# Illumina/canvas

Hardware: AMD Instinct MI355X
Metric: genome-bins/sec (bin+clean+partition) (higher is better)
Workload: dtype u8/int32 (bin), f32/f64 (clean, viterbi); 1 GPU; BASELINE configs[2]: whole-genome GRCh38 60x single sample, full bin+clean+partition HIP path on 1 MI355X per sample; bins_after_clean=4686240, bin_size=534, partition=PerSampleHMM, clean_flags=-g -s -r --local-sd-metric-file, segments=250, samples=1

## Files before the change

### canvas_amd/csrc/hmm.hip

```cpp
#include "common.hpp"
#include <type_traits>
#include "select.hpp"
#include "quantize.hpp"
#include <mutex>
#include <cmath>
#include <thread>
#include <cstring>
#include <limits>
#include <algorithm>

#define NSTATE 5

struct HmmParams {
    double logA[NSTATE][NSTATE];
    double logPi[NSTATE];
    int32_t tableLen;
    double maxThreshold;
};

__global__ void __launch_bounds__(256) k_keys_cov_f32(const double* __restrict__ cov, int64_t n, uint32_t* __restrict__ keys) {
    int64_t i = (int64_t)blockIdx.x * 256 + threadIdx.x;
    if (i < n) keys[i] = key_of_float((float)cov[i]);
}

// ... 409 lines not shown
#pragma unroll
            for (int j = 0; j < NSTATE; j++) { d[j] = on ? dn[j] : d[j]; eCur[j] = eNext[j]; }
            if (WM) { fm = (on && s >= lead) ? map_compose(fm, pk) : fm; pks[u] = pk; }
        }
        if (WM) {
#pragma unroll
            for (int u = 0; u < PQ; u++) { const int s = s0 + u; if (s < nsteps && s >= lead) pp[ts + s] = (uint16_t)pks[u]; }
        }
        qa = na; qb = nb;
    };
    const int leadMin = -wave_max_i32(nsteps > 0 ? -lead : -0x7FFFFFFF);
    int s0 = 1;
    for (; s0 + PQ <= leadMin && s0 < maxSteps; s0 += PQ) group(s0, std::false_type{});
    for (; s0 < maxSteps; s0 += PQ) group(s0, std::true_type{});
    if (act) {
        maps[b] = (uint16_t)fm;
        if (tEnd == C.T) lastGuess[B.chrom] = vit_best5(d);
    }
}

#define CHR_LDS_CAP 1024
__device__ __forceinline__ const int64_t* stage_chr_offsets(const int64_t* __restrict__ chrOff, int nchr, int64_t* sOff) {
    if (nchr + 1 > CHR_LDS_CAP) return chrOff;
    for (int k = threadIdx.x; k <= nchr; k += blockDim.x) sOff[k] = chrOff[k];
    __syncthreads();
    return sOff;
}
__device__ __forceinline__ int chrom_of_bin(const int64_t* off, int nchr, int64_t g) {
    int lo = 0, hi = nchr - 1;
    while (lo < hi) { const int mid = (lo + hi + 1) >> 1; if (off[mid] <= g) lo = mid; else hi = mid - 1; }
    return lo;
}
#define VBS (VB / 2)
__global__ void __launch_bounds__(256) k_pair_maps(const VitBlock* __restrict__ blocks, int nblocks, const HmmChrom* __restrict__ chroms, const int32_t* __restrict__ firstS,
                                                   const uint16_t* __restrict__ mapsS, uint16_t* __restrict__ maps, const int32_t* __restrict__ todo) {
    const int b = blockIdx.x * 256 + threadIdx.x;
    if (b >= nblocks) return;
    const VitBlock B = blocks[b];
    if (todo && !todo[B.chrom]) return;
    const int64_t T = chroms[B.chrom].T;
    const int s0 = firstS[B.chrom] + B.t0 / VBS;
    uint32_t m = mapsS[s0];
#pragma unroll
    for (int k = 1; k < VB / VBS; k++) if (B.t0 + (int64_t)k * VBS < T) m = map_compose(m, mapsS[s0 + k]);
    maps[b] = (uint16_t)m;
}

__global__ void __launch_bounds__(256) k_vit_increments(const HmmChrom* __restrict__ chroms, int nchr, const int64_t* __restrict__ chrOff, const int32_t* __restrict__ idx,
                                                        const double* __restrict__ logPmf, HmmParams P, const int32_t* __restrict__ state, int64_t N, double* __restrict__ D) {
    __shared__ int64_t sOff[CHR_LDS_CAP];
    const int64_t* off = stage_chr_offsets(chrOff, nchr, sOff);
    int64_t g = (int64_t)blockIdx.x * 256 + threadIdx.x;
    if (g >= N) return;
    const int s1 = state[g], sPrev = state[g > 0 ? g - 1 : 0], ix = idx[g];
    const int lo = chrom_of_bin(off, nchr, g);
    const int64_t begin = chroms[lo].begin;
    if (s1 < 0) { D[g] = 0.0; return; }
    double e = logPmf[(size_t)s1 * P.tableLen + ix];
    if (g == begin) { double lik = e + P.logA[0][s1]; D[g] = P.logPi[s1] + lik - P.logA[0][s1]; }
    else { const int s0 = sPrev; D[g] = e + P.logA[s0 < 0 ? 0 : s0][s1]; }
}

__global__ void __launch_bounds__(64) k_vit_backbone(const HmmChrom* __restrict__ chroms, const double* __restrict__ V, double* __restrict__ carryOut, const int32_t* __restrict__ todo = nullptr) {
    __shared__ double sV[2][64];
    const HmmChrom C = chroms[blockIdx.x];
    if (C.T <= 10 || (todo && !todo[blockIdx.x])) return;
    const int l = threadIdx.x;
    const double* __restrict__ Vc = V + C.begin;
    double acc = 0.0;
    double vNext = l < C.T ? Vc[l] : 0.0;
    int buf = 0;
    for (int64_t c0 = 0; c0 < C.T; c0 += 64, buf ^= 1) {
        sV[buf][l] = vNext;
        { int64_t t2 = c0 + 64 + l; vNext = t2 < C.T ? Vc[t2] : 0.0; }
        if (l == 0) carryOut[C.begin + c0] = acc;
        double r[64];
#pragma unroll
        for (int s = 0; s < 64; s++) r[s] = sV[buf][s];
#pragma unroll
        for (int s = 0; s < 64; s++) acc = acc + r[s];
    }
}

#define BS_T 1024
#define BS_I 8
struct ParFn { unsigned long long a0, a1; };
__device__ __forceinline__ ParFn parfn_then(ParFn f, ParFn g) {
    ParFn h;
    h.a0 = f.a0 + ((f.a0 & 1ull) ? g.a1 : g.a0);
    h.a1 = f.a1 + ((f.a1 & 1ull) ? g.a0 : g.a1);
    return h;
}
__device__ __forceinline__ ParFn parfn_shfl_up(ParFn f, int d) {
// ... 93 lines not shown
        }
        __syncthreads();
        if (cross < chunkEnd && myCross == cross) {
            const double Mprev = __longlong_as_double((long long)(expBits | (kBefore & MANT)));
            const double acc = -Mprev + Vc[cross];
            if (((cross + 1) & 63) == 0 && cross + 1 < C.T) carry[cross + 1] = acc;
            sM = -acc; sP = cross + 1; sCross = 0x7fffffffffffffffll;
        }
        __syncthreads();
    }
}

#define BB_CHUNK 1024
#define BB_MAXC 16
struct BbChunk { int32_t chrom; int32_t t0; };
struct BbCross { ParFn before; double v; int32_t pos; int32_t e; };
struct BbChunkOut { ParFn tail; int32_t nCross; int32_t headE; int64_t pad; };
struct BbPost { unsigned long long bits; };
__device__ __forceinline__ bool bb_bad_increment(unsigned long long vb) { return ((vb >> 52) & 0x7ffull) == 0x7ffull || (!(vb >> 63) && (vb << 1) != 0ull); }
__device__ __forceinline__ ParFn parfn_of(unsigned long long vb, int eM) {
    const unsigned long long MANT = (1ull << 52) - 1ull;
    const int ea = (int)((vb >> 52) & 0x7ffull);
    const unsigned long long ma = ea ? ((vb & MANT) | (1ull << 52)) : (vb & MANT);
    const int shift = eM - (ea ? ea : 1);
    unsigned long long A = 0; int r = 0;
    if (shift <= 0) { if (ma) A = 1ull << 53; }
    else if (shift < 64) { A = ma >> shift; const unsigned long long rem = ma & ((1ull << shift) - 1ull), half = 1ull << (shift - 1); r = rem > half ? 1 : (rem == half ? 2 : 0); }
    const unsigned long long up = A + (r == 1 ? 1ull : 0ull);
    ParFn f; f.a0 = up + ((r == 2 && (A & 1ull)) ? 1ull : 0ull); f.a1 = up + ((r == 2 && !(A & 1ull)) ? 1ull : 0ull);
    return f;
}
__device__ __forceinline__ double shfl_up_f64(double v, int d) { return __hiloint2double(__shfl_up(__double2hiint(v), d), __shfl_up(__double2loint(v), d)); }

__global__ void __launch_bounds__(256) k_bb_sums(const BbChunk* __restrict__ chunks, const HmmChrom* __restrict__ chroms, const double* __restrict__ V, double* __restrict__ chunkSum,
                                                 int32_t* __restrict__ fail) {
    __shared__ double sw[4];
    const BbChunk K = chunks[blockIdx.x];
    const HmmChrom C = chroms[K.chrom];
    const double* __restrict__ Vc = V + C.begin;
    double s = 0.0; bool bad = false;
#pragma unroll
    for (int i = 0; i < 4; i++) {
        const int64_t t = (int64_t)K.t0 + threadIdx.x * 4 + i;
        if (t < C.T) { const double v = Vc[t]; bad |= bb_bad_increment((unsigned long long)__double_as_longlong(v)); s += fabs(v); }
    }
#pragma unroll
    for (int d = 32; d >= 1; d >>= 1) s += __hiloint2double(__shfl_xor(__double2hiint(s), d), __shfl_xor(__double2loint(s), d));
    if ((threadIdx.x & 63) == 0) sw[threadIdx.x >> 6] = s;
    if (bad) fail[K.chrom] = 1;
    __syncthreads();
    if (threadIdx.x == 0) chunkSum[blockIdx.x] = (sw[0] + sw[1]) + (sw[2] + sw[3]);
}
__global__ void __launch_bounds__(64) k_bb_bases(const int32_t* __restrict__ firstChunk, const double* __restrict__ chunkSum, double* __restrict__ chunkBase) {
    const int c = blockIdx.x, l = threadIdx.x;
    double carry = 0.0;
    for (int g = firstChunk[c]; g < firstChunk[c + 1]; g += 64) {
        const int i = g + l;
        const double v = i < firstChunk[c + 1] ? chunkSum[i] : 0.0;
        double inc = v;
#pragma unroll
        for (int d = 1; d < 64; d <<= 1) { double o = shfl_up_f64(inc, d); if (l >= d) inc += o; }
        if (i < firstChunk[c + 1]) chunkBase[i] = carry + (inc - v);
        carry += __hiloint2double(__builtin_amdgcn_readlane(__double2hiint(inc), 63), __builtin_amdgcn_readlane(__double2loint(inc), 63));
    }
}
struct SegFn { ParFn f; uint32_t head; uint32_t cnt; };
__device__ __forceinline__ SegFn segfn_then(SegFn a, SegFn b) {
    SegFn r; r.head = a.head | b.head; r.cnt = a.cnt + b.cnt; r.f = b.head ? b.f : parfn_then(a.f, b.f);
    return r;
}
__global__ void __launch_bounds__(256) k_bb_pieces(const BbChunk* __restrict__ chunks, const HmmChrom* __restrict__ chroms, const double* __restrict__ V,
                                                   const double* __restrict__ chunkBase, BbChunkOut* __restrict__ outChunk, BbCross* __restrict__ outCross,
                                                   ParFn* __restrict__ at64Fn, uint8_t* __restrict__ at64Rank, int32_t* __restrict__ fail) {
    __shared__ double swSum[4];
    __shared__ SegFn swSeg[4];
    const BbChunk K = chunks[blockIdx.x];
    const HmmChrom C = chroms[K.chrom];
// ... 282 lines not shown
            double e[NSTATE];
            vit_emissions(e, sTab, logPmf, useLds, P.tableLen, ix[0]);
            const double Dt = S.Dprev + Vc[0];
            const int sCur = st[0];
            vit_init5(S.d, e, P); S.valid = 31u;
            if (sel5(S.d, (uint32_t)sCur) != Dt) { S.bad = true; S.why |= 16u; }
            S.Dprev = Dt; S.sPrev = sCur;
        } else ver_lead_step<useLds>(S, A, sTab, logPmf, P.tableLen, true, ix[0], st[0], Vc[0], (uint32_t)pp[0]);
    }
    const int start2 = lead > 1 ? lead : 1;
    ver_phase<useLds, true>(S, A, P, sTab, logPmf, ix + 1, st + 1, Vc + 1, pp + 1, nsteps > 0 && lead > 1 ? lead - 1 : 0);
    ver_phase<useLds, false>(S, A, P, sTab, logPmf, ix + start2, st + start2, Vc + start2, pp + start2, nsteps > start2 ? nsteps - start2 : 0);
    double (&d)[NSTATE] = S.d; const uint32_t valid = S.valid; bool bad = S.bad;
    uint32_t why = S.why;
    if (act && tEnd == C.T) { if (valid != 31u || vit_best5(d) != lastGuess[B.chrom]) { bad = true; why |= 32u; } }
    if (act && bad) atomicOr(&fail[B.chrom], (int32_t)(1u | why));
}

__global__ void k_vit_corrupt(uint16_t* __restrict__ psi, int64_t at, int j) {
    if (threadIdx.x == 0 && blockIdx.x == 0) { const uint32_t sh = 3u * (uint32_t)j; uint32_t v = psi[at], p = (v >> sh) & 7u; psi[at] = (uint16_t)((v & ~(7u << sh)) | (((p + 1u) % 5u) << sh)); }
}

__global__ void __launch_bounds__(256) k_bt_maps(const VitBlock* __restrict__ blocks, int nblocks, const HmmChrom* __restrict__ chroms, const uint16_t* __restrict__ psi,
                                                 uint16_t* __restrict__ maps) {
    int b = blockIdx.x * 256 + threadIdx.x;
    if (b >= nblocks) return;
    const VitBlock B = blocks[b];
    const HmmChrom C = chroms[B.chrom];
    const int64_t tBeg = B.t0 > 0 ? B.t0 : 1, tEnd = (B.t0 + VB < C.T) ? B.t0 + VB : C.T;
    uint32_t m = MAP_IDENT;
    for (int64_t t = tEnd - 1; t >= tBeg; t--) m = map_compose(psi[C.begin + t], m);
    maps[b] = (uint16_t)m;
}
__global__ void __launch_bounds__(64) k_bt_group(const int32_t* __restrict__ firstBlock, const int32_t* __restrict__ firstGroup, int nchr, const uint16_t* __restrict__ maps,
                                                 uint16_t* __restrict__ pre, uint16_t* __restrict__ gmap) {
    const int g = blockIdx.x, l = threadIdx.x;
    int lo = 0, hi = nchr - 1;
    while (lo < hi) { const int mid = (lo + hi + 1) >> 1; if (firstGroup[mid] <= g) lo = mid; else hi = mid - 1; }
    while (lo < nchr - 1 && firstGroup[lo + 1] <= g) lo++;
    const int first = firstBlock[lo], last = firstBlock[lo + 1] - 1;
    const int bi = last - ((g - firstGroup[lo]) * 64 + l);
    uint32_t f = bi >= first ? (uint32_t)maps[bi] : MAP_IDENT;
#pragma unroll
    for (int dlt = 1; dlt < 64; dlt <<= 1) { const uint32_t o = __shfl_up(f, dlt); if (l >= dlt) f = map_compose(f, o); }
    const uint32_t ex = __shfl_up(f, 1);
    if (bi >= first) pre[bi] = (uint16_t)(l == 0 ? MAP_IDENT : ex);
    if (l == 63) gmap[g] = (uint16_t)f;
}
__global__ void __launch_bounds__(64) k_bt_gchain(const int32_t* __restrict__ firstGroup, const int32_t* __restrict__ lastState, const uint16_t* __restrict__ gmap,
                                                  int8_t* __restrict__ gentry) {
    const int c = blockIdx.x, l = threadIdx.x;
    const int g0 = firstGroup[c], ng = firstGroup[c + 1] - g0;
    int s = lastState[c];
    for (int base = 0; base < ng; base += 64) {
        uint32_t f = base + l < ng ? (uint32_t)gmap[g0 + base + l] : MAP_IDENT;
#pragma unroll
        for (int dlt = 1; dlt < 64; dlt <<= 1) { const uint32_t o = __shfl_up(f, dlt); if (l >= dlt) f = map_compose(f, o); }
        const uint32_t ex = __shfl_up(f, 1);
        if (base + l < ng) gentry[g0 + base + l] = (int8_t)(s < 0 ? s : (l == 0 ? s : (int)map_get(ex, (uint32_t)s)));
        const uint32_t all = (uint32_t)__builtin_amdgcn_readlane((int)f, 63);
        if (s >= 0) s = (int)map_get(all, (uint32_t)s);
    }
}
__global__ void __launch_bounds__(256) k_bt_states(const VitBlock* __restrict__ blocks, int nblocks, const HmmChrom* __restrict__ chroms, const uint16_t* __restrict__ psi,
                                                   const int32_t* __restrict__ firstBlock, const int32_t* __restrict__ firstGroup, const uint16_t* __restrict__ pre,
                                                   const int8_t* __restrict__ gentry, int32_t* __restrict__ state) {
    static_assert(VB <= 128, "two steps per lane");
    const int b = blockIdx.x * 4 + (threadIdx.x >> 6), l = lane_id();
    if (b >= nblocks) return;
    const VitBlock B = blocks[b];
    const HmmChrom C = chroms[B.chrom];
    const int64_t tBeg = B.t0, tEnd = (B.t0 + VB < C.T) ? B.t0 + VB : C.T;
    const int cnt = (int)(tEnd - tBeg);
    const int sg = gentry[firstGroup[B.chrom] + (firstBlock[B.chrom + 1] - 1 - b) / 64];
    const int s = sg < 0 ? sg : (int)map_get((uint32_t)pre[b], (uint32_t)sg);
// ... 285 lines not shown
        L.firstBlock[c] = L.nblocks;
        if (L.chroms[c].T > 10) L.nblocks += (int)((L.chroms[c].T + VB - 1) / VB);
    }
    L.firstBlock[nchr] = L.nblocks;
    L.firstGroup.resize(nchr + 1);
    for (int c = 0; c < nchr; c++) { L.firstGroup[c] = L.ngroups; L.ngroups += (L.firstBlock[c + 1] - L.firstBlock[c] + 63) / 64; }
    L.firstGroup[nchr] = L.ngroups;
    L.firstS.resize(nchr + 1);
    for (int c = 0; c < nchr; c++) { L.firstS[c] = L.nblocksS; if (L.chroms[c].T > 10) L.nblocksS += (int)((L.chroms[c].T + VBS - 1) / VBS); }
    L.firstS[nchr] = L.nblocksS;
    L.firstChunk.resize(nchr + 1);
    for (int c = 0; c < nchr; c++) {
        L.firstChunk[c] = L.nchunks;
        if (L.chroms[c].T > 10) L.nchunks += (int)((L.chroms[c].T + BB_CHUNK - 1) / BB_CHUNK);
    }
    L.firstChunk[nchr] = L.nchunks;
    return L;
}

enum { BB_MODE_CHAIN = 0, BB_MODE_SCAN = 1, BB_MODE_PIECES = 2 };
struct BbWork { double* chunkSum; double* chunkBase; BbChunkOut* chunkOut; BbCross* cross; ParFn* at64Fn; uint8_t* at64Rank; unsigned long long* chunkBits; BbPost* post; };
static void bb_work_size(WsSizer& sz, int nchunks) {
    sz.take<double>(nchunks + 1); sz.take<double>(nchunks + 1); sz.take<BbChunkOut>(nchunks + 1);
    sz.take<BbCross>((size_t)nchunks * BB_MAXC + 1); sz.take<ParFn>((size_t)nchunks * 16 + 1); sz.take<uint8_t>((size_t)nchunks * 16 + 8);
    sz.take<unsigned long long>(nchunks + 1); sz.take<BbPost>((size_t)nchunks * BB_MAXC + 1);
}
static BbWork bb_work_carve(WsCarver& ws, int nchunks) {
    BbWork W;
    W.chunkSum = ws.take<double>(nchunks + 1); W.chunkBase = ws.take<double>(nchunks + 1); W.chunkOut = ws.take<BbChunkOut>(nchunks + 1);
    W.cross = ws.take<BbCross>((size_t)nchunks * BB_MAXC + 1); W.at64Fn = ws.take<ParFn>((size_t)nchunks * 16 + 1); W.at64Rank = ws.take<uint8_t>((size_t)nchunks * 16 + 8);
    W.chunkBits = ws.take<unsigned long long>(nchunks + 1); W.post = ws.take<BbPost>((size_t)nchunks * BB_MAXC + 1);
    return W;
}
static void enqueue_backbone(canvas_ctx* ctx, int mode, int nchr, int nchunks, const HmmChrom* dChroms, const BbChunk* dBChunks, const int32_t* dFirstChunk, const double* dV,
                             double* dCarry, int32_t* dFail, const int32_t* dTodo, const BbWork& W) {
    if (mode == BB_MODE_CHAIN) hipLaunchKernelGGL(k_vit_backbone, dim3(nchr), dim3(64), 0, ctx->stream, dChroms, dV, dCarry, dTodo);
    else if (mode == BB_MODE_SCAN) hipLaunchKernelGGL(k_vit_backbone_scan, dim3(nchr), dim3(BS_T), 0, ctx->stream, dChroms, dV, dCarry, dFail);
    else {
        hipLaunchKernelGGL(k_bb_sums, dim3(nchunks), dim3(256), 0, ctx->stream, dBChunks, dChroms, dV, W.chunkSum, dFail);
        hipLaunchKernelGGL(k_bb_bases, dim3(nchr), dim3(64), 0, ctx->stream, dFirstChunk, W.chunkSum, W.chunkBase);
        hipLaunchKernelGGL(k_bb_pieces, dim3(nchunks), dim3(256), 0, ctx->stream, dBChunks, dChroms, dV, W.chunkBase, W.chunkOut, W.cross, W.at64Fn, W.at64Rank, dFail);
        hipLaunchKernelGGL(k_bb_walk, dim3(nchr), dim3(64), 0, ctx->stream, dFirstChunk, W.chunkOut, W.cross, W.chunkBits, W.post, dFail);
        hipLaunchKernelGGL(k_bb_emit, dim3(nblk2((int64_t)nchunks * 16, 256)), dim3(256), 0, ctx->stream, dBChunks, nchunks, dChroms, W.chunkBits, W.post, W.at64Fn, W.at64Rank, dCarry);
    }
}

struct VitCorrupt { bool on = false, retry = false; int chrom = 0; int64_t t = 0; int state = 2; int attempts = 0; };
static int32_t vit_corrupt_parse(canvas_ctx* ctx, int32_t nchr, const int64_t* h_chr_offset, VitCorrupt& K) {
    const char* s = cvx_hook("CANVAS_HMM_TEST_CORRUPT");
    if (!s) return CANVAS_OK;
    K.on = true;
    if (!strcmp(s, "1")) {
        const int64_t T = h_chr_offset[1] - h_chr_offset[0];
        K.chrom = 0; K.t = T / 2; K.state = 2; K.attempts = T > 10 ? 1 : 0;
        return CANVAS_OK;
    }
    long long v[4] = {0, 0, 0, 0}; int nf = 0; const char* p = s;
    for (;;) {
        char* end = nullptr;
        if (nf == 4 || *p < '0' || *p > '9') { nf = -1; break; }
        v[nf++] = strtoll(p, &end, 10);
        if (end - p > 12) { nf = -1; break; }
        if (*end == 0) break;
        if (*end != ':') { nf = -1; break; }
        p = end + 1;
    }
    if (nf != 3 && nf != 4) CANVAS_FAIL(ctx, CANVAS_ERR_INVALID, "CANVAS_HMM_TEST_CORRUPT: 1, c:t:j or c:t:j:k");
    if (v[0] >= nchr) CANVAS_FAIL(ctx, CANVAS_ERR_INVALID, "CANVAS_HMM_TEST_CORRUPT: no such chromosome");
    const int64_t T = h_chr_offset[v[0] + 1] - h_chr_offset[v[0]];
    if (T <= 10 || v[1] < 1 || v[1] >= T) CANVAS_FAIL(ctx, CANVAS_ERR_INVALID, "CANVAS_HMM_TEST_CORRUPT: the step must be 1 .. T-1 of a chromosome of more than ten bins");
    if (v[2] >= NSTATE) CANVAS_FAIL(ctx, CANVAS_ERR_INVALID, "CANVAS_HMM_TEST_CORRUPT: the state must be 0 .. 4");
    if (nf == 4 && (v[3] < 1 || v[3] > 5)) CANVAS_FAIL(ctx, CANVAS_ERR_INVALID, "CANVAS_HMM_TEST_CORRUPT: 1 .. 5 corrupted attempts");
    K.chrom = (int)v[0]; K.t = v[1]; K.state = (int)v[2]; K.attempts = nf == 4 ? (int)v[3] : 1; K.retry = nf == 4;
    return CANVAS_OK;
}

struct HmmEmis { int32_t* idx = nullptr; double* dTab = nullptr;
                 const double* indexCov = nullptr; };
struct SegPost { const int32_t* d_start; const int32_t* d_stop; int32_t maxDist; int32_t* d_segment_id; int64_t nseg = 0; bool valid = false; };
static void enqueue_segment_ids(canvas_ctx* ctx, const int64_t* dOff, int nchr, const int32_t* d_state, const int32_t* d_start, const int32_t* d_stop, int64_t N, int32_t maxDist,
                                uint8_t* flags, uint32_t* blockCnt, unsigned long long* dTot, int32_t* d_segment_id, unsigned* totSeq = nullptr, unsigned seq = 0);
template <class PrepareA, class PrepareB>
static int32_t hmm_pipeline(canvas_ctx* ctx, int32_t nchr, const int64_t* h_chr_offset, size_t extraBytes, PrepareA prepareA, PrepareB prepareB, int32_t* d_state, SegPost* seg = nullptr,
                            bool descByValue = false ) {
    const int64_t N = h_chr_offset[nchr];
    VitCorrupt corrupt;
    { int32_t rcc = vit_corrupt_parse(ctx, nchr, h_chr_offset, corrupt); if (rcc) return rcc; }
    const HmmLists L = hmm_lists(nchr, h_chr_offset);
    const std::vector<HmmChrom>& chroms = L.chroms;
    const std::vector<int32_t>&firstBlock = L.firstBlock, &firstGroup = L.firstGroup, &firstS = L.firstS, &firstChunk = L.firstChunk;
    const int nblocks = L.nblocks, ngroups = L.ngroups, nblocksS = L.nblocksS, nchunks = L.nchunks;
    const int nbSeg = (int)nblk2(N, 2048);
    WsSizer sz;
    sz.take<BbChunk>(nchunks + 1); sz.take<int32_t>(nchr + 1); bb_work_size(sz, nchunks);
    sz.take<uint16_t>(N + 8); sz.take<HmmChrom>(nchr); sz.take<int32_t>(nchr);
    sz.take<int32_t>(nchr + 1); sz.take<uint16_t>(nblocks + 8); sz.take<int8_t>(nblocks + 8);
    sz.take<int64_t>(nchr + 1); sz.take<VitBlock>(nblocks + 1); sz.take<double>(N); sz.take<double>(N + 64); sz.take<int32_t>(nchr); sz.take<int32_t>(nchr);
    sz.take<VitBlock>(nblocksS + 1); sz.take<uint16_t>(nblocksS + 8); sz.take<int32_t>(nchr + 1);
    sz.take<int32_t>(nchr + 1); sz.take<uint16_t>(nblocks + 8); sz.take<uint16_t>(ngroups + 8); sz.take<int8_t>(ngroups + 8);
    sz.take<char>(8 * 256 + (size_t)nchr * 64 + 64);
    if (seg) { sz.take<uint8_t>(N + 16); sz.take<uint32_t>(nbSeg + 1); sz.take<unsigned long long>(1); }
    int32_t rc = canvas_ws_reserve(ctx, sz.off + extraBytes + 65536); if (rc) return rc;
    rc = canvas_pin_reserve(ctx, (size_t)nchr * 4 + 64); if (rc) return rc;
    WsCarver ws(ctx->ws);
    uint16_t* psi = ws.take<uint16_t>(N + 8);
    HmmChrom* dChroms = ws.take<HmmChrom>(nchr); int32_t* dLast = ws.take<int32_t>(nchr);
    int32_t* dFirst = ws.take<int32_t>(nchr + 1);
    uint16_t* dMaps = ws.take<uint16_t>(nblocks + 8); (void)ws.take<int8_t>(nblocks + 8);
    int64_t* dOffDev = ws.take<int64_t>(nchr + 1);
    VitBlock* dVBlocks = ws.take<VitBlock>(nblocks + 1); double* dD = ws.take<double>(N); double* dCarry = ws.take<double>(N + 64); int32_t* dFail = ws.take<int32_t>(nchr); int32_t* dRedo = ws.take<int32_t>(nchr);
    int32_t* dFirstGroup = ws.take<int32_t>(nchr + 1); uint16_t* dPre = ws.take<uint16_t>(nblocks + 8); uint16_t* dGmap = ws.take<uint16_t>(ngroups + 8);
    int8_t* dGentry = ws.take<int8_t>(ngroups + 8);
    VitBlock* dSBlocks = ws.take<VitBlock>(nblocksS + 1); uint16_t* dMapsS = ws.take<uint16_t>(nblocksS + 8); int32_t* dFirstS = ws.take<int32_t>(nchr + 1);
    BbChunk* dBChunks = ws.take<BbChunk>(nchunks + 1); int32_t* dFirstChunk = ws.take<int32_t>(nchr + 1);
// ... 12 lines not shown
            memset(&pack, 0, sizeof pack);
            memcpy(pack.chroms, chroms.data(), (size_t)nchr * sizeof(HmmChrom)); memcpy(pack.off, h_chr_offset, (size_t)(nchr + 1) * 8); memcpy(pack.first, firstBlock.data(), (size_t)(nchr + 1) * 4);
            memcpy(pack.firstChunk, firstChunk.data(), (size_t)(nchr + 1) * 4); memcpy(pack.firstS, firstS.data(), (size_t)(nchr + 1) * 4); memcpy(pack.firstGroup, firstGroup.data(), (size_t)(nchr + 1) * 4);
        } else {
            std::vector<char> blob(total, 0);
            memcpy(blob.data() + oCh, chroms.data(), (size_t)nchr * sizeof(HmmChrom)); memcpy(blob.data() + oFirst, firstBlock.data(), (size_t)(nchr + 1) * 4);
            memcpy(blob.data() + oOff, h_chr_offset, (size_t)(nchr + 1) * 8); memcpy(blob.data() + oChunk, firstChunk.data(), (size_t)(nchr + 1) * 4);
            memcpy(blob.data() + oS, firstS.data(), (size_t)(nchr + 1) * 4); memcpy(blob.data() + oG, firstGroup.data(), (size_t)(nchr + 1) * 4);
            rc = canvas_h2d_small(ctx, dBlob, blob.data(), total); if (rc) return rc;
        }
        dChroms = (HmmChrom*)(dBlob + oCh); dFirst = (int32_t*)(dBlob + oFirst); dOffDev = (int64_t*)(dBlob + oOff); dFirstChunk = (int32_t*)(dBlob + oChunk);
        dFirstS = (int32_t*)(dBlob + oS); dFirstGroup = (int32_t*)(dBlob + oG);
    }
    HmmParams P; HmmEmis E;
    ctx->hmm_dispersion = 1e9;
    rc = prepareA(ws, P, E, (const HmmChrom*)dChroms, (const int64_t*)dOffDev); if (rc) return rc;
    {
        const int64_t most = std::max<int64_t>(std::max<int64_t>(E.indexCov ? N : 0, nblocks), std::max<int64_t>(std::max(nblocksS, nchunks), nchr));
        HmmDescDev DD{dChroms, dOffDev, dFirst, dFirstChunk, dFirstS, dFirstGroup};
        hipLaunchKernelGGL((k_hmm_setup<VitBlock, BbChunk>), dim3(nblk2(most, 256)), dim3(256), 0, ctx->stream, pack, byVal ? 1 : 0, DD, nchr, nblocks, nblocksS, nchunks, VB, VBS, BB_CHUNK,
                           dVBlocks, dSBlocks, dBChunks, E.indexCov, N, P.maxThreshold, E.idx, dLast, dFail);
    }
    rc = prepareB(ws, P, E); if (rc) return rc;
    int32_t* idx = E.idx; double* dTab = E.dTab;
    size_t tabBytes = (size_t)NSTATE * P.tableLen * 8;
    size_t lds = tabBytes <= 48 * 1024 ? tabBytes : 0;
    for (int c = 0; c < nchr; c++)
        if (chroms[c].T <= 10 && chroms[c].T > 0)
            hipLaunchKernelGGL(k_fill_i32, dim3(nblk2(chroms[c].T, 256)), dim3(256), 0, ctx->stream, d_state, chroms[c].begin, chroms[c].begin + chroms[c].T, -1);
    const unsigned laneGrid = (unsigned)((nblocks + 63) / 64);
    auto backtrack = [&](bool haveMaps) {
        if (nblocks > 0) {
            if (!haveMaps) hipLaunchKernelGGL(k_bt_maps, dim3(nblk2(nblocks, 256)), dim3(256), 0, ctx->stream, dVBlocks, nblocks, dChroms, psi, dMaps);
            hipLaunchKernelGGL(k_bt_group, dim3(ngroups), dim3(64), 0, ctx->stream, dFirst, dFirstGroup, nchr, dMaps, dPre, dGmap);
            hipLaunchKernelGGL(k_bt_gchain, dim3(nchr), dim3(64), 0, ctx->stream, dFirstGroup, dLast, dGmap, dGentry);
            hipLaunchKernelGGL(k_bt_states, dim3(nblk2(nblocks, 4)), dim3(256), 0, ctx->stream, dVBlocks, nblocks, dChroms, psi, dFirst, dFirstGroup, dPre, dGentry, d_state);
        }
    };
    bool twoValuedAll = true;
    for (int i = 0; i < NSTATE; i++) for (int j = 0; j < NSTATE; j++) {
        const double ref = i == j ? P.logA[0][0] : P.logA[0][1];
        if (memcmp(&P.logA[i][j], &ref, sizeof(double)) != 0) twoValuedAll = false;
    }
    const bool speculative = cvx_hook("CANVAS_HMM_SEQUENTIAL") == nullptr;
    std::vector<int32_t> redo;
    int32_t* hFail = (int32_t*)ctx->pin; unsigned long long* hSegTot = (unsigned long long*)((char*)ctx->pin + (((size_t)nchr * 4 + 15) & ~size_t(15)));
    bool segEnqueued = false; unsigned* hSegSeq = (unsigned*)(hSegTot + 1); unsigned segSeq = 0;
    if (speculative && nblocks > 0) {
        ProfScope ps(ctx, "viterbi");
        const int32_t* dTodo = nullptr;
        ctx->hmm_retry = 0;
        const int vwEnv = cvx_hook("CANVAS_HMM_LEAD") ? atoi(cvx_hook("CANVAS_HMM_LEAD")) : 0;
        const int vw0 = vwEnv > 0 ? vwEnv : (ctx->hmm_dispersion < 0.20 ? VW0 : (ctx->hmm_dispersion < 0.30 ? 64 : VW));
        const int nAttempts = 5;
        for (int attempt = 0; attempt < nAttempts; attempt++) {
            const int mult = attempt <= 1 ? 1 : (attempt == 2 ? 8 : (attempt == 3 ? 64 : 512));
            const int leadSpec = attempt == 0 ? vw0 : mult * VW, leadVer = mult * VW2;
            cvx_prof_count(ctx, "viterbi_attempt");
            if (attempt > 0) CANVAS_HIP_TRY(ctx, hipMemsetAsync(dFail, 0, nchr * 4, ctx->stream));
            const dim3 gs((unsigned)((nblocksS + 63) / 64));
            const bool twoValued = twoValuedAll && attempt < 3;
            if (lds && twoValued) hipLaunchKernelGGL((k_vit_spec<true, true>), gs, dim3(64), lds, ctx->stream, dSBlocks, nblocksS, dChroms, idx, dTab, P, psi, dMapsS, dLast, leadSpec, dTodo, VBS);
            else if (lds) hipLaunchKernelGGL((k_vit_spec<true, false>), gs, dim3(64), lds, ctx->stream, dSBlocks, nblocksS, dChroms, idx, dTab, P, psi, dMapsS, dLast, leadSpec, dTodo, VBS);
            else if (twoValued) hipLaunchKernelGGL((k_vit_spec<false, true>), gs, dim3(64), 0, ctx->stream, dSBlocks, nblocksS, dChroms, idx, dTab, P, psi, dMapsS, dLast, leadSpec, dTodo, VBS);
            else hipLaunchKernelGGL((k_vit_spec<false, false>), gs, dim3(64), 0, ctx->stream, dSBlocks, nblocksS, dChroms, idx, dTab, P, psi, dMapsS, dLast, leadSpec, dTodo, VBS);
            hipLaunchKernelGGL(k_pair_maps, dim3(nblk2(nblocks, 256)), dim3(256), 0, ctx->stream, dVBlocks, nblocks, dChroms, dFirstS, dMapsS, dMaps, dTodo);
            if (attempt < corrupt.attempts) hipLaunchKernelGGL(k_vit_corrupt, dim3(1), dim3(64), 0, ctx->stream, psi, chroms[corrupt.chrom].begin + corrupt.t, corrupt.state);
            backtrack(true);
            hipLaunchKernelGGL(k_vit_increments, dim3(nblk2(N, 256)), dim3(256), 0, ctx->stream, dChroms, nchr, dOffDev, idx, dTab, P, d_state, N, dD);
            const char* bbMode = cvx_hook("CANVAS_HMM_BACKBONE");
            const int bb = ((bbMode && !strcmp(bbMode, "chain")) || (attempt > 1 && !bbMode)) ? BB_MODE_CHAIN : ((bbMode && !strcmp(bbMode, "scan")) ? BB_MODE_SCAN : BB_MODE_PIECES);
            enqueue_backbone(ctx, bb, nchr, nchunks, dChroms, dBChunks, dFirstChunk, dD, dCarry, dFail, dTodo, bbWork);
            if (lds) hipLaunchKernelGGL((k_vit_verify<true>), dim3(laneGrid), dim3(64), lds, ctx->stream, dVBlocks, nblocks, dChroms, idx, dTab, P, psi, d_state, dD, dCarry, dLast, dFail, leadVer, dTodo);
            else hipLaunchKernelGGL((k_vit_verify<false>), dim3(laneGrid), dim3(64), 0, ctx->stream, dVBlocks, nblocks, dChroms, idx, dTab, P, psi, d_state, dD, dCarry, dLast, dFail, leadVer, dTodo);
            CANVAS_HIP_TRY(ctx, hipMemcpyAsync(hFail, dFail, nchr * 4, hipMemcpyDeviceToHost, ctx->stream));
            if (seg && attempt == 0 && (!corrupt.on || corrupt.retry)) {
                (void)segTot;
                segSeq = cvx_mail_arm(ctx, hSegSeq);
                enqueue_segment_ids(ctx, dOffDev, nchr, d_state, seg->d_start, seg->d_stop, N, seg->maxDist, segFlags, segBlockCnt, hSegTot , seg->d_segment_id, hSegSeq, segSeq);
                segEnqueued = true;
            }
            CANVAS_HIP_TRY(ctx, hipStreamSynchronize(ctx->stream));
            redo.clear();
            for (int c = 0; c < nchr; c++) if (hFail[c] && chroms[c].T > 10) redo.push_back(c);
            if (!redo.empty() && cvx_hook("CANVAS_HMM_DEBUG_FAIL")) { fprintf(stderr, "viterbi attempt %d (lead-in x%d):", attempt, mult); for (int c : redo) fprintf(stderr, " chr%d(T=%lld, why=0x%x)", c, (long long)chroms[c].T, (unsigned)hFail[c]); fprintf(stderr, "\n"); }
            if (redo.empty() || (corrupt.on && !corrupt.retry) || cvx_hook("CANVAS_HMM_NO_RETRY")) break;
            if (attempt < nAttempts - 1) {
                if (attempt == 0) { ctx->hmm_retry = (int)redo.size(); { ProfScope pr(ctx, "viterbi_retry"); } }
                int32_t rcq = canvas_h2d_small(ctx, dRedo, hFail, nchr * 4); if (rcq) return rcq;
                dTodo = dRedo;
            }
        }
        if (seg && segEnqueued && redo.empty() && ctx->hmm_retry == 0) { int32_t rcm = cvx_mail_await(ctx, hSegSeq, segSeq, "PerSampleHMM: segment count"); if (rcm) return rcm; seg->valid = true; seg->nseg = (int64_t)*hSegTot; }
    } else {
        for (int c = 0; c < nchr; c++) redo.push_back(c);
    }
    if (!redo.empty()) {
        const bool isFallback = speculative && nblocks > 0;
        ProfScope ps(ctx, isFallback ? "viterbi_sequential" : "viterbi_small");
        if (cvx_hook("CANVAS_HMM_DEBUG_FAIL")) { fprintf(stderr, "viterbi sequential kernel for %zu chromosomes (speculative %d, blocks %d):", redo.size(), (int)speculative, nblocks); for (size_t i = 0; i < redo.size() && i < 6; i++) fprintf(stderr, " chr%d(T=%lld)", redo[i], (long long)chroms[redo[i]].T); fprintf(stderr, "\n"); }
        rc = canvas_h2d_small(ctx, dRedo, redo.data(), redo.size() * 4); if (rc) return rc;
        hipLaunchKernelGGL(k_viterbi, dim3((unsigned)redo.size()), dim3(64), lds, ctx->stream, dChroms, idx, dTab, P, psi, dLast, dRedo);
        backtrack(false);
    }
    ctx->hmm_redo = (int)redo.size();
    CANVAS_HIP_TRY(ctx, hipStreamSynchronize(ctx->stream));
    CANVAS_HIP_TRY(ctx, hipGetLastError());
    return CANVAS_OK;
}

extern "C" {

static int32_t hmm_per_sample_impl(canvas_ctx* ctx, int32_t nchr, const double* d_cov, const int64_t* h_chr_offset, const double* d_cov_all, int64_t nAll, int32_t* d_state, const CovQ* preQ = nullptr, SegPost* seg = nullptr) {
    if (!ctx) return CANVAS_ERR_INVALID;
// ... 240 lines not shown
    return hmm_pipeline(ctx, nchr, h_chr_offset, ex.off, prepare, [](WsCarver&, HmmParams&, HmmEmis&) -> int32_t { return CANVAS_OK; }, d_state);
}

extern "C" int32_t canvas_hmm_backbone_probe(canvas_ctx* ctx, int32_t mode, int32_t nchr, const int64_t* h_chr_offset, const double* d_V, double* d_carry, int32_t* h_fail) {
    if (!ctx) return CANVAS_ERR_INVALID;
    if (mode < BB_MODE_CHAIN || mode > BB_MODE_PIECES || nchr < 1 || nchr > (1 << 20) || !h_chr_offset || !h_fail)
        CANVAS_FAIL(ctx, CANVAS_ERR_INVALID, "canvas_hmm_backbone_probe: bad arguments (mode 0..2, 1..2^20 chromosomes)");
    if (h_chr_offset[0] != 0) CANVAS_FAIL(ctx, CANVAS_ERR_INVALID, "canvas_hmm_backbone_probe: the offsets start at 0");
    for (int c = 0; c < nchr; c++) if (h_chr_offset[c + 1] < h_chr_offset[c] || h_chr_offset[c + 1] > (1ll << 30)) CANVAS_FAIL(ctx, CANVAS_ERR_INVALID, "canvas_hmm_backbone_probe: the offsets decrease or pass 2^30 steps");
    const int64_t N = h_chr_offset[nchr];
    if (N > 0 && (!d_V || !d_carry)) CANVAS_FAIL(ctx, CANVAS_ERR_INVALID, "canvas_hmm_backbone_probe: no increments / no room for the carries");
    for (int c = 0; c < nchr; c++) h_fail[c] = 0;
    const HmmLists L = hmm_lists(nchr, h_chr_offset);
    const int nchunks = L.nchunks;
    if (nchunks == 0) return CANVAS_OK;
    CANVAS_HIP_TRY(ctx, hipSetDevice(ctx->device));
    WsSizer sz; sz.take<HmmChrom>(nchr); sz.take<int32_t>(nchr + 1); sz.take<BbChunk>(nchunks + 1); sz.take<int32_t>(nchr); bb_work_size(sz, nchunks);
    int32_t rc = canvas_ws_reserve(ctx, sz.off + 65536); if (rc) return rc;
    WsCarver ws(ctx->ws);
    HmmChrom* dChroms = ws.take<HmmChrom>(nchr); int32_t* dFirstChunk = ws.take<int32_t>(nchr + 1); BbChunk* dBChunks = ws.take<BbChunk>(nchunks + 1); int32_t* dFail = ws.take<int32_t>(nchr);
    const BbWork W = bb_work_carve(ws, nchunks);
    rc = canvas_h2d_small(ctx, dChroms, L.chroms.data(), (size_t)nchr * sizeof(HmmChrom)); if (rc) return rc;
    rc = canvas_h2d_small(ctx, dFirstChunk, L.firstChunk.data(), (size_t)(nchr + 1) * 4); if (rc) return rc;
    CANVAS_HIP_TRY(ctx, hipMemsetAsync(dFail, 0, (size_t)nchr * 4, ctx->stream));
    hipLaunchKernelGGL((k_make_blocks<BbChunk>), dim3(nblk2(nchunks, 256)), dim3(256), 0, ctx->stream, dFirstChunk, nchr, nchunks, BB_CHUNK, dBChunks);
    enqueue_backbone(ctx, mode, nchr, nchunks, dChroms, dBChunks, dFirstChunk, d_V, d_carry, dFail, nullptr, W);
    CANVAS_HIP_TRY(ctx, hipGetLastError());
    CANVAS_HIP_TRY(ctx, hipStreamSynchronize(ctx->stream));
    CANVAS_HIP_TRY(ctx, hipMemcpy(h_fail, dFail, (size_t)nchr * 4, hipMemcpyDeviceToHost));
    return CANVAS_OK;
}

static void enqueue_segment_ids(canvas_ctx* ctx, const int64_t* dOff, int nchr, const int32_t* d_state, const int32_t* d_start, const int32_t* d_stop, int64_t N, int32_t maxDist,
                                uint8_t* flags, uint32_t* blockCnt, unsigned long long* dTot, int32_t* d_segment_id, unsigned* totSeq, unsigned seq) {
    const int nb = (int)nblk2(N, 2048);
    hipLaunchKernelGGL(k_seg_flags, dim3(nblk2(N, 256)), dim3(256), 0, ctx->stream, dOff, nchr, d_state, d_start, d_stop, N, maxDist, (const int64_t*)nullptr, (const int32_t*)nullptr, (const int32_t*)nullptr,
                       (const int64_t*)nullptr, (const int32_t*)nullptr, (const int32_t*)nullptr, (const int32_t*)nullptr, flags);
    hipLaunchKernelGGL(k_count_blocks, dim3(nb), dim3(256), 0, ctx->stream, flags, N, blockCnt);
    hipLaunchKernelGGL(k_scan_blocks2, dim3(1), dim3(1024), 0, ctx->stream, blockCnt, nb, dTot, totSeq, seq);
    hipLaunchKernelGGL(k_seg_ids, dim3(nb), dim3(256), 0, ctx->stream, flags, blockCnt, N, d_segment_id);
}
extern "C" {
int32_t canvas_segment_ids_ploidy(canvas_ctx* ctx, int32_t nchr, const int64_t* h_chr_offset, const int32_t* d_state, const int32_t* d_start,
                                  const int32_t* d_stop, int32_t max_inter_bin_dist, const int64_t* h_excl_offset, const int32_t* h_excl_start,
                                  const int32_t* h_excl_stop, const int64_t* h_ploidy_offset, const int32_t* h_ploidy_start, const int32_t* h_ploidy_end,
                                  const int32_t* h_ploidy_cn, int32_t* d_segment_id, int64_t* h_nsegments) {
    if (!ctx) return CANVAS_ERR_INVALID;
    if (nchr <= 0 || !h_chr_offset || !d_state || !d_start || !d_stop || !d_segment_id) CANVAS_FAIL(ctx, CANVAS_ERR_INVALID, "canvas_segment_ids: bad arguments");
    CANVAS_HIP_TRY(ctx, hipSetDevice(ctx->device));
    const int64_t N = h_chr_offset[nchr];
    if (N == 0) { if (h_nsegments) *h_nsegments = 0; return CANVAS_OK; }
    const int nb = (int)nblk2(N, 2048);
    const int64_t nex = h_excl_offset ? h_excl_offset[nchr] : 0;
    if (h_excl_offset && nex > 0 && (!h_excl_start || !h_excl_stop)) CANVAS_FAIL(ctx, CANVAS_ERR_INVALID, "canvas_segment_ids_filtered: missing interval arrays");
    if (h_excl_offset) for (int c = 0; c < nchr; c++) for (int64_t k = h_excl_offset[c] + 1; k < h_excl_offset[c + 1]; k++)
        if (h_excl_stop[k] < h_excl_stop[k - 1]) CANVAS_FAIL(ctx, CANVAS_ERR_UNSUPPORTED, "forbidden intervals must be sorted by end within a chromosome");
    const int64_t npl = h_ploidy_offset ? h_ploidy_offset[nchr] : 0;
    if (h_ploidy_offset && npl > 0 && (!h_ploidy_start || !h_ploidy_end || !h_ploidy_cn)) CANVAS_FAIL(ctx, CANVAS_ERR_INVALID, "canvas_segment_ids_ploidy: missing ploidy arrays");
    for (int64_t k = 0; k < npl; k++) if (h_ploidy_cn[k] < 0 || h_ploidy_cn[k] > 4)
        CANVAS_FAIL(ctx, CANVAS_ERR_INVALID, "reference ploidy outside 0..4 (PloidyInfo.getPloidyCounts indexes a 5-element array: the reference throws)");
    WsSizer sz; sz.take<int64_t>(nchr + 1); sz.take<uint8_t>(N); sz.take<uint32_t>(nb + 1); sz.take<unsigned long long>(1);
    sz.take<int64_t>(nchr + 1); sz.take<int32_t>(nex + 1); sz.take<int32_t>(nex + 1);
    sz.take<int64_t>(nchr + 1); sz.take<int32_t>(npl + 1); sz.take<int32_t>(npl + 1); sz.take<int32_t>(npl + 1);
    int32_t rc = canvas_ws_reserve(ctx, sz.off + 4096); if (rc) return rc;
    WsCarver ws(ctx->ws);
    int64_t* dOff = ws.take<int64_t>(nchr + 1); uint8_t* flags = ws.take<uint8_t>(N); uint32_t* blockCnt = ws.take<uint32_t>(nb + 1); unsigned long long* dTot = ws.take<unsigned long long>(1);
    int64_t* dExOff = ws.take<int64_t>(nchr + 1); int32_t* dExStart = ws.take<int32_t>(nex + 1); int32_t* dExStop = ws.take<int32_t>(nex + 1);
    int64_t* dPlOff = ws.take<int64_t>(nchr + 1); int32_t* dPlStart = ws.take<int32_t>(npl + 1); int32_t* dPlEnd = ws.take<int32_t>(npl + 1); int32_t* dPlCn = ws.take<int32_t>(npl + 1);
    if (h_ploidy_offset) {
        CANVAS_HIP_TRY(ctx, hipMemcpyAsync(dPlOff, h_ploidy_offset, (nchr + 1) * 8, hipMemcpyHostToDevice, ctx->stream));
        if (npl > 0) { CANVAS_HIP_TRY(ctx, hipMemcpyAsync(dPlStart, h_ploidy_start, npl * 4, hipMemcpyHostToDevice, ctx->stream));
                       CANVAS_HIP_TRY(ctx, hipMemcpyAsync(dPlEnd, h_ploidy_end, npl * 4, hipMemcpyHostToDevice, ctx->stream));
                       CANVAS_HIP_TRY(ctx, hipMemcpyAsync(dPlCn, h_ploidy_cn, npl * 4, hipMemcpyHostToDevice, ctx->stream)); }
// ... 55 lines not shown
```

Measured before the change: 1.933 billion bins/s.

## Fuse Viterbi increments into backbone sums, pair maps into bt_group, overlap segmentation

Computes the Viterbi log-likelihood increments inside k_bb_sums for the pieces backbone, dropping the separate k_vit_increments pass and its extra read of D. It also folds the pair-map composition into k_bt_group, so the k_pair_maps kernel and the dMaps round trip are gone. Segment-id computation now runs on a side stream forked after backtracking and is joined before the host sync, so it overlaps the backbone and verify kernels. In exchange this adds stream and event management with a join guard, and k_bt_group does more work per lane.

```diff
diff --git a/canvas_amd/csrc/hmm.hip b/canvas_amd/csrc/hmm.hip
--- a/canvas_amd/csrc/hmm.hip
+++ b/canvas_amd/csrc/hmm.hip
@@ -465,20 +465,14 @@
     return lo;
 }
 #define VBS (VB / 2)
-__global__ void __launch_bounds__(256) k_pair_maps(const VitBlock* __restrict__ blocks, int nblocks, const HmmChrom* __restrict__ chroms, const int32_t* __restrict__ firstS,
-                                                   const uint16_t* __restrict__ mapsS, uint16_t* __restrict__ maps, const int32_t* __restrict__ todo) {
-    const int b = blockIdx.x * 256 + threadIdx.x;
-    if (b >= nblocks) return;
-    const VitBlock B = blocks[b];
-    if (todo && !todo[B.chrom]) return;
-    const int64_t T = chroms[B.chrom].T;
-    const int s0 = firstS[B.chrom] + B.t0 / VBS;
-    uint32_t m = mapsS[s0];
-#pragma unroll
-    for (int k = 1; k < VB / VBS; k++) if (B.t0 + (int64_t)k * VBS < T) m = map_compose(m, mapsS[s0 + k]);
-    maps[b] = (uint16_t)m;
-}
-
+
+__device__ __forceinline__ double vit_increment(const double* __restrict__ logPmf, const HmmParams& P, int s1, int sPrev, int ix, bool first) {
+    if (s1 < 0) return 0.0;
+    const double e = logPmf[(size_t)s1 * P.tableLen + ix];
+    if (first) { const double lik = e + P.logA[0][s1]; return P.logPi[s1] + lik - P.logA[0][s1]; }
+    const int s0 = sPrev;
+    return e + P.logA[s0 < 0 ? 0 : s0][s1];
+}
 __global__ void __launch_bounds__(256) k_vit_increments(const HmmChrom* __restrict__ chroms, int nchr, const int64_t* __restrict__ chrOff, const int32_t* __restrict__ idx,
                                                         const double* __restrict__ logPmf, HmmParams P, const int32_t* __restrict__ state, int64_t N, double* __restrict__ D) {
     __shared__ int64_t sOff[CHR_LDS_CAP];
@@ -488,10 +482,7 @@
     const int s1 = state[g], sPrev = state[g > 0 ? g - 1 : 0], ix = idx[g];
     const int lo = chrom_of_bin(off, nchr, g);
     const int64_t begin = chroms[lo].begin;
-    if (s1 < 0) { D[g] = 0.0; return; }
-    double e = logPmf[(size_t)s1 * P.tableLen + ix];
-    if (g == begin) { double lik = e + P.logA[0][s1]; D[g] = P.logPi[s1] + lik - P.logA[0][s1]; }
-    else { const int s0 = sPrev; D[g] = e + P.logA[s0 < 0 ? 0 : s0][s1]; }
+    D[g] = vit_increment(logPmf, P, s1, sPrev, ix, g == begin);
 }
 
 __global__ void __launch_bounds__(64) k_vit_backbone(const HmmChrom* __restrict__ chroms, const double* __restrict__ V, double* __restrict__ carryOut, const int32_t* __restrict__ todo = nullptr) {
@@ -651,17 +642,44 @@
 }
 __device__ __forceinline__ double shfl_up_f64(double v, int d) { return __hiloint2double(__shfl_up(__double2hiint(v), d), __shfl_up(__double2loint(v), d)); }
 
+template <bool FORM>
 __global__ void __launch_bounds__(256) k_bb_sums(const BbChunk* __restrict__ chunks, const HmmChrom* __restrict__ chroms, const double* __restrict__ V, double* __restrict__ chunkSum,
-                                                 int32_t* __restrict__ fail) {
+                                                 int32_t* __restrict__ fail, const int32_t* __restrict__ state = nullptr, const int32_t* __restrict__ idx = nullptr,
+                                                 const double* __restrict__ logPmf = nullptr, HmmParams P = HmmParams(), double* __restrict__ Vout = nullptr) {
     __shared__ double sw[4];
     const BbChunk K = chunks[blockIdx.x];
     const HmmChrom C = chroms[K.chrom];
     const double* __restrict__ Vc = V + C.begin;
     double s = 0.0; bool bad = false;
+    const int64_t t0 = (int64_t)K.t0 + threadIdx.x * 4;
+    double vf[4] = {0.0, 0.0, 0.0, 0.0};
+    if (FORM && t0 < C.T) {
+        const int32_t* __restrict__ st = state + C.begin + t0; const int32_t* __restrict__ ix = idx + C.begin + t0;
+        int sq[5], kq[4];
+        sq[0] = t0 > 0 ? st[-1] : -1;
+        if (t0 + 4 <= C.T) {
+            const VecI4 sa = *reinterpret_cast<const VecI4*>(st), ka = *reinterpret_cast<const VecI4*>(ix);
+#pragma unroll
+            for (int i = 0; i < 4; i++) { sq[1 + i] = sa.v[i]; kq[i] = ka.v[i]; }
+        } else {
+#pragma unroll
+            for (int i = 0; i < 4; i++) { const bool in = t0 + i < C.T; sq[1 + i] = in ? st[i] : -1; kq[i] = in ? ix[i] : 0; }
+        }
+#pragma unroll
+        for (int i = 0; i < 4; i++) vf[i] = vit_increment(logPmf, P, sq[1 + i], sq[i], kq[i], t0 + i == 0);
+        double* __restrict__ vo = Vout + C.begin + t0;
+        if (t0 + 4 <= C.T) {
+            VecD2 a, b; a.v[0] = vf[0]; a.v[1] = vf[1]; b.v[0] = vf[2]; b.v[1] = vf[3];
+            *reinterpret_cast<VecD2*>(vo) = a; *reinterpret_cast<VecD2*>(vo + 2) = b;
+        } else {
+#pragma unroll
+            for (int i = 0; i < 4; i++) if (t0 + i < C.T) vo[i] = vf[i];
+        }
+    }
 #pragma unroll
     for (int i = 0; i < 4; i++) {
-        const int64_t t = (int64_t)K.t0 + threadIdx.x * 4 + i;
-        if (t < C.T) { const double v = Vc[t]; bad |= bb_bad_increment((unsigned long long)__double_as_longlong(v)); s += fabs(v); }
+        const int64_t t = t0 + i;
+        if (t < C.T) { const double v = FORM ? vf[i] : Vc[t]; bad |= bb_bad_increment((unsigned long long)__double_as_longlong(v)); s += fabs(v); }
     }
 #pragma unroll
     for (int d = 32; d >= 1; d >>= 1) s += __hiloint2double(__shfl_xor(__double2hiint(s), d), __shfl_xor(__double2loint(s), d));
@@ -1010,15 +1028,25 @@
     for (int64_t t = tEnd - 1; t >= tBeg; t--) m = map_compose(psi[C.begin + t], m);
     maps[b] = (uint16_t)m;
 }
+template <bool PAIR>
 __global__ void __launch_bounds__(64) k_bt_group(const int32_t* __restrict__ firstBlock, const int32_t* __restrict__ firstGroup, int nchr, const uint16_t* __restrict__ maps,
-                                                 uint16_t* __restrict__ pre, uint16_t* __restrict__ gmap) {
+                                                 uint16_t* __restrict__ pre, uint16_t* __restrict__ gmap, const HmmChrom* __restrict__ chroms = nullptr, const int32_t* __restrict__ firstS = nullptr) {
     const int g = blockIdx.x, l = threadIdx.x;
     int lo = 0, hi = nchr - 1;
     while (lo < hi) { const int mid = (lo + hi + 1) >> 1; if (firstGroup[mid] <= g) lo = mid; else hi = mid - 1; }
     while (lo < nchr - 1 && firstGroup[lo + 1] <= g) lo++;
     const int first = firstBlock[lo], last = firstBlock[lo + 1] - 1;
     const int bi = last - ((g - firstGroup[lo]) * 64 + l);
-    uint32_t f = bi >= first ? (uint32_t)maps[bi] : MAP_IDENT;
+    uint32_t f = MAP_IDENT;
+    if (PAIR) {
+        if (bi >= first) {
+            const int64_t T = chroms[lo].T, t0 = (int64_t)(bi - first) * VB;
+            const int s0 = firstS[lo] + (bi - first) * (VB / VBS);
+            f = maps[s0];
+#pragma unroll
+            for (int k = 1; k < VB / VBS; k++) if (t0 + (int64_t)k * VBS < T) f = map_compose(f, maps[s0 + k]);
+        }
+    } else if (bi >= first) f = (uint32_t)maps[bi];
 #pragma unroll
     for (int dlt = 1; dlt < 64; dlt <<= 1) { const uint32_t o = __shfl_up(f, dlt); if (l >= dlt) f = map_compose(f, o); }
     const uint32_t ex = __shfl_up(f, 1);
@@ -1370,12 +1398,14 @@
     W.chunkBits = ws.take<unsigned long long>(nchunks + 1); W.post = ws.take<BbPost>((size_t)nchunks * BB_MAXC + 1);
     return W;
 }
+struct BbForm { const int32_t* state; const int32_t* idx; const double* logPmf; const HmmParams* P; double* V; };
 static void enqueue_backbone(canvas_ctx* ctx, int mode, int nchr, int nchunks, const HmmChrom* dChroms, const BbChunk* dBChunks, const int32_t* dFirstChunk, const double* dV,
-                             double* dCarry, int32_t* dFail, const int32_t* dTodo, const BbWork& W) {
+                             double* dCarry, int32_t* dFail, const int32_t* dTodo, const BbWork& W, const BbForm* form = nullptr) {
     if (mode == BB_MODE_CHAIN) hipLaunchKernelGGL(k_vit_backbone, dim3(nchr), dim3(64), 0, ctx->stream, dChroms, dV, dCarry, dTodo);
     else if (mode == BB_MODE_SCAN) hipLaunchKernelGGL(k_vit_backbone_scan, dim3(nchr), dim3(BS_T), 0, ctx->stream, dChroms, dV, dCarry, dFail);
     else {
-        hipLaunchKernelGGL(k_bb_sums, dim3(nchunks), dim3(256), 0, ctx->stream, dBChunks, dChroms, dV, W.chunkSum, dFail);
+        if (form) hipLaunchKernelGGL((k_bb_sums<true>), dim3(nchunks), dim3(256), 0, ctx->stream, dBChunks, dChroms, dV, W.chunkSum, dFail, form->state, form->idx, form->logPmf, *form->P, form->V);
+        else hipLaunchKernelGGL((k_bb_sums<false>), dim3(nchunks), dim3(256), 0, ctx->stream, dBChunks, dChroms, dV, W.chunkSum, dFail);
         hipLaunchKernelGGL(k_bb_bases, dim3(nchr), dim3(64), 0, ctx->stream, dFirstChunk, W.chunkSum, W.chunkBase);
         hipLaunchKernelGGL(k_bb_pieces, dim3(nchunks), dim3(256), 0, ctx->stream, dBChunks, dChroms, dV, W.chunkBase, W.chunkOut, W.cross, W.at64Fn, W.at64Rank, dFail);
         hipLaunchKernelGGL(k_bb_walk, dim3(nchr), dim3(64), 0, ctx->stream, dFirstChunk, W.chunkOut, W.cross, W.chunkBits, W.post, dFail);
@@ -1417,7 +1447,7 @@
                  const double* indexCov = nullptr; };
 struct SegPost { const int32_t* d_start; const int32_t* d_stop; int32_t maxDist; int32_t* d_segment_id; int64_t nseg = 0; bool valid = false; };
 static void enqueue_segment_ids(canvas_ctx* ctx, const int64_t* dOff, int nchr, const int32_t* d_state, const int32_t* d_start, const int32_t* d_stop, int64_t N, int32_t maxDist,
-                                uint8_t* flags, uint32_t* blockCnt, unsigned long long* dTot, int32_t* d_segment_id, unsigned* totSeq = nullptr, unsigned seq = 0);
+                                uint8_t* flags, uint32_t* blockCnt, unsigned long long* dTot, int32_t* d_segment_id, hipStream_t stream, unsigned* totSeq = nullptr, unsigned seq = 0);
 template <class PrepareA, class PrepareB>
 static int32_t hmm_pipeline(canvas_ctx* ctx, int32_t nchr, const int64_t* h_chr_offset, size_t extraBytes, PrepareA prepareA, PrepareB prepareB, int32_t* d_state, SegPost* seg = nullptr,
                             bool descByValue = false ) {
@@ -1496,7 +1526,8 @@
     auto backtrack = [&](bool haveMaps) {
         if (nblocks > 0) {
             if (!haveMaps) hipLaunchKernelGGL(k_bt_maps, dim3(nblk2(nblocks, 256)), dim3(256), 0, ctx->stream, dVBlocks, nblocks, dChroms, psi, dMaps);
-            hipLaunchKernelGGL(k_bt_group, dim3(ngroups), dim3(64), 0, ctx->stream, dFirst, dFirstGroup, nchr, dMaps, dPre, dGmap);
+            if (haveMaps) hipLaunchKernelGGL((k_bt_group<true>), dim3(ngroups), dim3(64), 0, ctx->stream, dFirst, dFirstGroup, nchr, dMapsS, dPre, dGmap, dChroms, dFirstS);
+            else hipLaunchKernelGGL((k_bt_group<false>), dim3(ngroups), dim3(64), 0, ctx->stream, dFirst, dFirstGroup, nchr, dMaps, dPre, dGmap);
             hipLaunchKernelGGL(k_bt_gchain, dim3(nchr), dim3(64), 0, ctx->stream, dFirstGroup, dLast, dGmap, dGentry);
             hipLaunchKernelGGL(k_bt_states, dim3(nblk2(nblocks, 4)), dim3(256), 0, ctx->stream, dVBlocks, nblocks, dChroms, psi, dFirst, dFirstGroup, dPre, dGentry, d_state);
         }
@@ -1510,6 +1541,18 @@
     std::vector<int32_t> redo;
     int32_t* hFail = (int32_t*)ctx->pin; unsigned long long* hSegTot = (unsigned long long*)((char*)ctx->pin + (((size_t)nchr * 4 + 15) & ~size_t(15)));
     bool segEnqueued = false; unsigned* hSegSeq = (unsigned*)(hSegTot + 1); unsigned segSeq = 0;
+    struct SideJoin {
+        canvas_ctx* ctx; bool forked = false;
+        int32_t join() {
+            if (!forked) return CANVAS_OK;
+            forked = false;
+            hipError_t e = hipStreamWaitEvent(ctx->stream, ctx->side_ev2, 0);
+            if (e != hipSuccess) { (void)hipStreamSynchronize(ctx->side); ctx->err = std::string("hipStreamWaitEvent(side_ev2): ") + hipGetErrorString(e); return CANVAS_ERR_HIP; }
+            return CANVAS_OK;
+        }
+        ~SideJoin() { if (forked) (void)hipStreamSynchronize(ctx->side); }
+    } sideJoin{ctx};
+    if (seg) { rc = canvas_side_init(ctx); if (rc) return rc; }
     if (speculative && nblocks > 0) {
         ProfScope ps(ctx, "viterbi");
         const int32_t* dTodo = nullptr;
@@ -1528,22 +1571,28 @@
             else if (lds) hipLaunchKernelGGL((k_vit_spec<true, false>), gs, dim3(64), lds, ctx->stream, dSBlocks, nblocksS, dChroms, idx, dTab, P, psi, dMapsS, dLast, leadSpec, dTodo, VBS);
             else if (twoValued) hipLaunchKernelGGL((k_vit_spec<false, true>), gs, dim3(64), 0, ctx->stream, dSBlocks, nblocksS, dChroms, idx, dTab, P, psi, dMapsS, dLast, leadSpec, dTodo, VBS);
             else hipLaunchKernelGGL((k_vit_spec<false, false>), gs, dim3(64), 0, ctx->stream, dSBlocks, nblocksS, dChroms, idx, dTab, P, psi, dMapsS, dLast, leadSpec, dTodo, VBS);
-            hipLaunchKernelGGL(k_pair_maps, dim3(nblk2(nblocks, 256)), dim3(256), 0, ctx->stream, dVBlocks, nblocks, dChroms, dFirstS, dMapsS, dMaps, dTodo);
             if (attempt < corrupt.attempts) hipLaunchKernelGGL(k_vit_corrupt, dim3(1), dim3(64), 0, ctx->stream, psi, chroms[corrupt.chrom].begin + corrupt.t, corrupt.state);
             backtrack(true);
-            hipLaunchKernelGGL(k_vit_increments, dim3(nblk2(N, 256)), dim3(256), 0, ctx->stream, dChroms, nchr, dOffDev, idx, dTab, P, d_state, N, dD);
+            if (seg && attempt == 0 && (!corrupt.on || corrupt.retry)) {
+                (void)segTot;
+                CANVAS_HIP_TRY(ctx, hipEventRecord(ctx->side_ev, ctx->stream));
+                CANVAS_HIP_TRY(ctx, hipStreamWaitEvent(ctx->side, ctx->side_ev, 0));
+                sideJoin.forked = true;
+                segSeq = cvx_mail_arm(ctx, hSegSeq);
+                enqueue_segment_ids(ctx, dOffDev, nchr, d_state, seg->d_start, seg->d_stop, N, seg->maxDist, segFlags, segBlockCnt, hSegTot , seg->d_segment_id,
+                                    ctx->side, hSegSeq, segSeq);
+                CANVAS_HIP_TRY(ctx, hipEventRecord(ctx->side_ev2, ctx->side));
+                segEnqueued = true;
+            }
             const char* bbMode = cvx_hook("CANVAS_HMM_BACKBONE");
             const int bb = ((bbMode && !strcmp(bbMode, "chain")) || (attempt > 1 && !bbMode)) ? BB_MODE_CHAIN : ((bbMode && !strcmp(bbMode, "scan")) ? BB_MODE_SCAN : BB_MODE_PIECES);
-            enqueue_backbone(ctx, bb, nchr, nchunks, dChroms, dBChunks, dFirstChunk, dD, dCarry, dFail, dTodo, bbWork);
+            const BbForm form{d_state, idx, dTab, &P, dD};
+            if (bb != BB_MODE_PIECES) hipLaunchKernelGGL(k_vit_increments, dim3(nblk2(N, 256)), dim3(256), 0, ctx->stream, dChroms, nchr, dOffDev, idx, dTab, P, d_state, N, dD);
+            enqueue_backbone(ctx, bb, nchr, nchunks, dChroms, dBChunks, dFirstChunk, dD, dCarry, dFail, dTodo, bbWork, bb == BB_MODE_PIECES ? &form : nullptr);
             if (lds) hipLaunchKernelGGL((k_vit_verify<true>), dim3(laneGrid), dim3(64), lds, ctx->stream, dVBlocks, nblocks, dChroms, idx, dTab, P, psi, d_state, dD, dCarry, dLast, dFail, leadVer, dTodo);
             else hipLaunchKernelGGL((k_vit_verify<false>), dim3(laneGrid), dim3(64), 0, ctx->stream, dVBlocks, nblocks, dChroms, idx, dTab, P, psi, d_state, dD, dCarry, dLast, dFail, leadVer, dTodo);
             CANVAS_HIP_TRY(ctx, hipMemcpyAsync(hFail, dFail, nchr * 4, hipMemcpyDeviceToHost, ctx->stream));
-            if (seg && attempt == 0 && (!corrupt.on || corrupt.retry)) {
-                (void)segTot;
-                segSeq = cvx_mail_arm(ctx, hSegSeq);
-                enqueue_segment_ids(ctx, dOffDev, nchr, d_state, seg->d_start, seg->d_stop, N, seg->maxDist, segFlags, segBlockCnt, hSegTot , seg->d_segment_id, hSegSeq, segSeq);
-                segEnqueued = true;
-            }
+            { int32_t rcj = sideJoin.join(); if (rcj) return rcj; }
             CANVAS_HIP_TRY(ctx, hipStreamSynchronize(ctx->stream));
             redo.clear();
             for (int c = 0; c < nchr; c++) if (hFail[c] && chroms[c].T > 10) redo.push_back(c);
@@ -1850,13 +1899,13 @@
 }
 
 static void enqueue_segment_ids(canvas_ctx* ctx, const int64_t* dOff, int nchr, const int32_t* d_state, const int32_t* d_start, const int32_t* d_stop, int64_t N, int32_t maxDist,
-                                uint8_t* flags, uint32_t* blockCnt, unsigned long long* dTot, int32_t* d_segment_id, unsigned* totSeq, unsigned seq) {
+                                uint8_t* flags, uint32_t* blockCnt, unsigned long long* dTot, int32_t* d_segment_id, hipStream_t stream, unsigned* totSeq, unsigned seq) {
     const int nb = (int)nblk2(N, 2048);
-    hipLaunchKernelGGL(k_seg_flags, dim3(nblk2(N, 256)), dim3(256), 0, ctx->stream, dOff, nchr, d_state, d_start, d_stop, N, maxDist, (const int64_t*)nullptr, (const int32_t*)nullptr, (const int32_t*)nullptr,
+    hipLaunchKernelGGL(k_seg_flags, dim3(nblk2(N, 256)), dim3(256), 0, stream, dOff, nchr, d_state, d_start, d_stop, N, maxDist, (const int64_t*)nullptr, (const int32_t*)nullptr, (const int32_t*)nullptr,
                        (const int64_t*)nullptr, (const int32_t*)nullptr, (const int32_t*)nullptr, (const int32_t*)nullptr, flags);
-    hipLaunchKernelGGL(k_count_blocks, dim3(nb), dim3(256), 0, ctx->stream, flags, N, blockCnt);
-    hipLaunchKernelGGL(k_scan_blocks2, dim3(1), dim3(1024), 0, ctx->stream, blockCnt, nb, dTot, totSeq, seq);
-    hipLaunchKernelGGL(k_seg_ids, dim3(nb), dim3(256), 0, ctx->stream, flags, blockCnt, N, d_segment_id);
+    hipLaunchKernelGGL(k_count_blocks, dim3(nb), dim3(256), 0, stream, flags, N, blockCnt);
+    hipLaunchKernelGGL(k_scan_blocks2, dim3(1), dim3(1024), 0, stream, blockCnt, nb, dTot, totSeq, seq);
+    hipLaunchKernelGGL(k_seg_ids, dim3(nb), dim3(256), 0, stream, flags, blockCnt, N, d_segment_id);
 }
 extern "C" {
 int32_t canvas_segment_ids_ploidy(canvas_ctx* ctx, int32_t nchr, const int64_t* h_chr_offset, const int32_t* d_state, const int32_t* d_start,
```

Measured after the change: 1.970 billion bins/s, median of 6. 1.9% higher.
